# XChenZ/havatar

Hardware: AMD Instinct MI355X
Metric: rendered frames/sec @512^2, 64 samples/ray (higher is better)
Workload: dtype f32 emulated, full-width operands: every operand = hi + lo fp16 + tail (= the fp32 value itself, >= 24 significant bits); the three leading partial products on v_mfma_f32_32x32x16_f16, the three terms of order 2^-22 (hi.tail, tail.hi, lo.lo) on block-scaled 4-/6-bit v_mfma_scale_f32_32x32x64_f8f6f4

## Files before the change

### havatar_amd/_lib.py

```python
import ctypes as C
import os

from . import switches

_HERE = os.path.dirname(os.path.abspath(__file__))
LIB_PATH = os.path.join(_HERE, "lib", "libhavatar_hip.so")

HAV_F32, HAV_F16, HAV_BF16, HAV_F64 = 0, 1, 2, 3
HAV_MLP_SPLIT_BF16, HAV_MLP_F32, HAV_MLP_SPLIT_F16, HAV_MLP_SPLIT_F16_MX = 0, 1, 2, 3
ABI_VERSION = 8
HAV_FLAG_PAIR_KERNEL, HAV_FLAG_FINE_CACHE, HAV_FLAG_FINE_RECOMPUTE, HAV_FLAG_NO_FP16_GUARD = 1, 2, 4, 8
HAV_STATUS_FP16_FALLBACK = 1


class HavRenderParams(C.Structure):
    _fields_ = [("B", C.c_int32), ("R", C.c_int32), ("ray_stride", C.c_int32), ("S_c", C.c_int32),
                ("S_f", C.c_int32), ("perturb", C.c_int32), ("noise_std", C.c_float),
                ("plane_res", C.c_int32), ("plane_ch", C.c_int32), ("vol_res", C.c_int32),
                ("nerf_scale", C.c_float * 3), ("nerf_trans", C.c_float * 3),
                ("skin_scale", C.c_float * 3), ("skin_trans", C.c_float * 3),
                ("seed", C.c_uint64), ("rng_offset", C.c_uint64), ("mlp_mode", C.c_int32), ("flags", C.c_int32),
                ("rng_counter", C.c_void_p), ("workspace", C.c_void_p), ("workspace_bytes", C.c_uint64),
                ("dbg_zfine", C.c_void_p), ("status", C.c_void_p), ("grid_blocks", C.c_int32), ("reserved0", C.c_int32)]

# ... 160 lines not shown
    L.hav_upsample3d_2x_fwd.restype = i32
    L.hav_upsample3d_2x_bwd.argtypes = [vp, vp, i64, i32, i32, i32, vp]
    for fn in (L.hav_im2col3d, L.hav_col2im3d):
        fn.argtypes = [vp, vp, i32, i32, vp]
        fn.restype = i32
    L.hav_upsample3d_2x_bwd.restype = i32
    L.hav_mlp_train_blob_bytes.restype = i64
    L.hav_mlp_train_ops_bytes.argtypes = [i64]
    L.hav_mlp_train_ops_bytes.restype = i64
    L.hav_mlp_train_partial_bytes.argtypes = [i64]
    L.hav_mlp_train_partial_bytes.restype = i64
    L.hav_mlp_train_pack.argtypes = [vp, C.POINTER(HavMlpWeights), vp]
    L.hav_mlp_train_pack.restype = i32
    L.hav_mlp_train_fwd.argtypes = [vp, vp, vp, i64, vp]
    L.hav_mlp_train_fwd.restype = i32
    L.hav_mlp_train_bwd.argtypes = [vp, C.POINTER(HavMlpGrads), i32, vp, vp, vp, vp, vp, i64, vp]
    L.hav_mlp_train_bwd.restype = i32
    L.hav_mlp_train_fwd_xbf16.argtypes = [vp, vp, vp, i64, vp]
    L.hav_mlp_train_fwd_xbf16.restype = i32
    L.hav_mlp_train_bwd_xbf16.argtypes = [vp, C.POINTER(HavMlpGrads), i32, vp, vp, vp, vp, vp, i64, vp]
    L.hav_mlp_train_bwd_xbf16.restype = i32
    L.hav_triplane_prepare.argtypes = [vp, vp, vp, i32, i32, i32, i32, vp]
    L.hav_triplane_prepare.restype = i32
    L.hav_triplane_prepared_bytes.argtypes = [i32, i32, i32]
    L.hav_triplane_prepared_bytes.restype = i64
    L.hav_render_rays.argtypes = [C.POINTER(HavRenderParams)] + [vp] * 10 + [C.POINTER(HavRenderOut), vp]
    L.hav_render_rays.restype = i32
    L.hav_render_workspace_bytes.argtypes = [C.POINTER(HavRenderParams)]
    L.hav_render_workspace_bytes.restype = i64
    L.hav_render_variant_name.argtypes = [C.POINTER(HavRenderParams), i32, i32, C.c_char_p, i32]
    L.hav_render_variant_name.restype = i32
    L.hav_gen_rays.argtypes = [vp, i32, i32, C.POINTER(f32), C.POINTER(f32), f32, f32, i32, i32, vp]
    L.hav_gen_rays.restype = i32
    L.hav_debug_mlp_layer.argtypes = [vp, vp, vp, i32, i32, i64, vp]
    L.hav_debug_mlp_layer.restype = i32
    L.hav_conv3d_k3_packed_bytes.argtypes = [i32, i32]
    L.hav_conv3d_k3_packed_bytes.restype = i64
    for fn in (L.hav_conv3d_k3_pack, L.hav_conv3d_k3_pack_t):
        fn.argtypes = [vp, vp, i32, i32, f32, vp]
        fn.restype = i32
    L.hav_conv3d_k3_scratch_bytes.argtypes = [i32] * 6
    L.hav_conv3d_k3_scratch_bytes.restype = i64
    L.hav_conv3d_k3_fwd.argtypes = [vp] * 5 + [i32] * 6 + [vp, vp]
    L.hav_conv3d_k3_fwd.restype = i32
    L.hav_conv3d_k3_wgrad_scratch_bytes.argtypes = [i32] * 6
    L.hav_conv3d_k3_wgrad_scratch_bytes.restype = i64
# ... 30 lines not shown
```

### havatar_amd/csrc/hav_render.hip

```cpp
#include "hav_common.h"
#include <stdio.h>
#include <stdlib.h>
#include <string.h>
#include <atomic>

#define HAV_HID 128
#define HAV_PC 64
#define HAV_IN (2 * HAV_PC + 48)
#define KPE_STEPS 24
#define K2_STEPS (HAV_HID / 2)
#define OFF_W1PE 0
#define OFF_W2 (OFF_W1PE + KPE_STEPS * 4 * 64)
#define OFF_W4 (OFF_W2 + K2_STEPS * 4 * 64)
#define OFF_WFT (OFF_W4 + K2_STEPS * 2 * 4)
#define LDS_FLOATS (OFF_WFT + HAV_HID * 64)
#define OFF_B1 LDS_FLOATS
#define OFF_B2 (OFF_B1 + 128)
#define OFF_B4 (OFF_B2 + 128)
#define OFF_BF (OFF_B4 + 4)
#define OFF_W1F (OFF_BF + 64)
#define OFF_WFF (OFF_W1F + 2 * 128 * 64)
#define OFF_A1S (OFF_WFF + K2_STEPS * 2 * 64)
#define OFF_A2S (OFF_A1S + 3 * 4 * 3 * 64 * 4)
#define OFF_W4S (OFF_A2S + 8 * 4 * 3 * 64 * 4)
// ... 225 lines not shown
        al[d] |= ql << o;
        if (o + 6 > 32) al[d + 1] |= ql >> (32 - o);
    }
    unsigned int* rec = reinterpret_cast<unsigned int*>(blob) + OFF_MX + G * MX_G_DWORDS;
    for (int d = 0; d < 4; ++d) { rec[l * 4 + d] = ah[d]; rec[256 + l * 4 + d] = at[d]; rec[512 + l * 4 + d] = al[d]; }
    rec[768 + l * 2 + 0] = al[4]; rec[768 + l * 2 + 1] = al[5];
    rec[896 + l] = (unsigned int)(sh + 127) | ((unsigned int)(st + 127) << 8) | ((unsigned int)(sl_ + 127) << 16);
}

extern "C" int hav_mlp_pack(void* blob, const HavMlpWeights* w, void* stream)
{
    if (!blob || !w || !w->W1 || !w->b1 || !w->W2 || !w->b2 || !w->Wa || !w->ba || !w->Wf || !w->bf || !w->Wc || !w->bc)
        return HAV_EINVAL;
    hipLaunchKernelGGL(mlp_pack_kernel, dim3((BLOB_FLOATS + 255) / 256), dim3(256), 0, (hipStream_t)stream, (float*)blob, *w);
    HAV_LAUNCH_CHECK();
    hipLaunchKernelGGL(mlp_wmax_kernel, dim3(1), dim3(256), 0, (hipStream_t)stream, (float*)blob, *w);
    HAV_LAUNCH_CHECK();
    hipLaunchKernelGGL(mlp_pack_mx_kernel, dim3(MX_GROUPS), dim3(64), 0, (hipStream_t)stream, (float*)blob, *w);
    HAV_LAUNCH_CHECK();
    return 0;
}

#define PREP_TRAILER_WORDS 512
__global__ void __launch_bounds__(256) plane_project_kernel(float* __restrict__ dst, const float* __restrict__ src,
                                                            const float* __restrict__ blob, int HW, unsigned int* __restrict__ trailer)
{
    extern __shared__ __attribute__((aligned(16))) float sm[];
    float* sX = sm;
    float* sW = sm + 64 * 64;
    float* sO = sW + 128 * 65;
    const int pb = blockIdx.y;
    const int p = pb / (gridDim.y / 2);
    const int t0 = blockIdx.x * 64;
    const int tid = threadIdx.x, tx = tid & 63, ty = tid >> 6;
    const float* plane = src + (size_t)pb * HAV_PC * HW;
    for (int c = ty; c < HAV_PC; c += 4) sX[c * 64 + tx] = (t0 + tx < HW) ? plane[(size_t)c * HW + t0 + tx] : 0.f;
    const float* wsrc = blob + OFF_W1F + (size_t)p * 128 * 64;
    for (int i = tid; i < 128 * 64; i += 256) sW[(i >> 6) * 65 + (i & 63)] = wsrc[i];
    __syncthreads();
    float acc[32];
#pragma unroll
    for (int o = 0; o < 32; ++o) acc[o] = 0.f;
    for (int c = 0; c < HAV_PC; ++c) {
        const float xv = sX[c * 64 + tx];
#pragma unroll
        for (int o = 0; o < 32; ++o) acc[o] = fmaf(sW[(ty * 32 + o) * 65 + c], xv, acc[o]);
    }
#pragma unroll
    for (int o = 0; o < 32; ++o) sO[tx * 129 + ty * 32 + o] = acc[o];
    __syncthreads();
    float* out = dst + (size_t)pb * HW * 128;
    const int tg = p ? HAV_TG1 : HAV_TG;
    if (t0 + 64 <= HW && (64 >> tg) << tg == 64) {
        float4* blk = reinterpret_cast<float4*>(out + (size_t)(t0 >> tg) * (128 << tg));
        for (int q = tid; q < 64 * 32; q += 256) {
            const int g = q / (32 << tg), rem = q - g * (32 << tg);
            const int piece = rem >> tg, tx4 = rem & ((1 << tg) - 1);
            const float* so = sO + ((g << tg) + tx4) * 129 + 4 * piece;
            blk[q] = make_float4(so[0], so[1], so[2], so[3]);
        }
    } else {
        for (int i = tid; i < 64 * 128; i += 256) {
            const int t = i >> 7, hu = i & 127;
            const int tt = t0 + t;
            if (tt < HW) out[(size_t)(tt >> tg) * (128 << tg) + (hu >> 2) * (4 << tg) + (tt & ((1 << tg) - 1)) * 4 + (hu & 3)] = sO[t * 129 + hu];
        }
    }
    if (tid < 128) {
        float m = 0.f;
        unsigned int bad = 0;
        for (int t = 0; t < 64; ++t) {
            const float x = fabsf(sO[t * 129 + tid]);
            bad |= (x != x);
            m = fmaxf(m, x);
        }
        atomicMax(&trailer[p * 128 + tid], bad ? 0x7FC00000u : __float_as_uint(m));
    }
}

__global__ void __launch_bounds__(128) range_verdict_kernel(unsigned int* __restrict__ trailer, const float* __restrict__ blob)
{
    __shared__ float b1u[128], red[128];
    const int t = threadIdx.x;
    {
        const float bound = blob[OFF_RNG + t] + __uint_as_float(trailer[t]) + __uint_as_float(trailer[128 + t]);
        b1u[acc_row((t & 63) >> 4, t & 15, t >> 6)] = bound;
        red[t] = (bound < HAV_FP16_LIMIT) ? bound : __builtin_inff();
    }
    __syncthreads();
    for (int st = 64; st > 0; st >>= 1) { if (t < st) red[t] = fmaxf(red[t], red[t + st]); __syncthreads(); }
    const float m1 = red[0];
    __syncthreads();
    {
        const int m = t >> 5, l31 = t & 31;
        float bound = fabsf(blob[OFF_B2 + t]);
        for (int ks = 0; ks < K2_STEPS; ++ks)
            for (int hh = 0; hh < 2; ++hh)
                bound += fabsf(blob[OFF_W2 + (ks * 4 + m) * 64 + hh * 32 + l31]) * b1u[acc_row(ks >> 4, ks & 15, hh)];
        red[t] = (bound < HAV_FP16_LIMIT) ? bound : __builtin_inff();
    }
    __syncthreads();
    for (int st = 64; st > 0; st >>= 1) { if (t < st) red[t] = fmaxf(red[t], red[t + st]); __syncthreads(); }
    if (t == 0) {
        const float m2 = red[0], wmax = blob[OFF_RNG + 128];
        const bool safe = (m1 < HAV_FP16_LIMIT) && (m2 < HAV_FP16_LIMIT) && (wmax < HAV_FP16_LIMIT);
        trailer[256] = safe ? 0u : 1u;
        trailer[257] = __float_as_uint(m1);
        trailer[258] = __float_as_uint(m2);
    }
}

extern "C" int64_t hav_triplane_prepared_bytes(int B, int H, int W) { return ((int64_t)2 * B * H * W * 128 + PREP_TRAILER_WORDS) * 4; }

static bool attr_done(std::atomic<unsigned long long>& mask, int& dev)
{
    dev = 0;
    if (hipGetDevice(&dev) != hipSuccess || dev < 0 || dev > 63) dev = 0;
    return (mask.load(std::memory_order_acquire) >> dev) & 1ull;
}

extern "C" int hav_triplane_prepare(float* dst, const float* src_nchw, const void* mlp_blob, int B, int C, int H, int W,
                                    void* stream)
{
    if (!dst || !src_nchw || !mlp_blob || B < 1 || H < 1 || W < 1) return HAV_EINVAL;
    if (C != HAV_PC || (W & ((1 << HAV_TG) - 1)) || (W & ((1 << HAV_TG1) - 1))) return HAV_EUNSUP;
    const int HW = H * W;
    const size_t lds = (64 * 64 + 128 * 65 + 64 * 129) * sizeof(float);
    static std::atomic<unsigned long long> attr_mask{0};
    int dev;
    if (!attr_done(attr_mask, dev)) {
        hipError_t e = hipFuncSetAttribute((const void*)plane_project_kernel, hipFuncAttributeMaxDynamicSharedMemorySize, (int)lds);
        if (e != hipSuccess) return (int)e;
        attr_mask.fetch_or(1ull << dev, std::memory_order_release);
    }
    unsigned int* trailer = reinterpret_cast<unsigned int*>(dst + (size_t)2 * B * HW * 128);
    hipError_t me = hipMemsetAsync(trailer, 0, PREP_TRAILER_WORDS * 4, (hipStream_t)stream);
    if (me != hipSuccess) return (int)me;
    hipLaunchKernelGGL(plane_project_kernel, dim3((HW + 63) / 64, 2 * B), dim3(256), lds, (hipStream_t)stream, dst, src_nchw,
                       (const float*)mlp_blob, HW, trailer);
    HAV_LAUNCH_CHECK();
    hipLaunchKernelGGL(range_verdict_kernel, dim3(1), dim3(128), 0, (hipStream_t)stream, trailer, (const float*)mlp_blob);
    HAV_LAUNCH_CHECK();
    return 0;
}

#define DPP_QUAD_XOR1 0xB1
#define DPP_QUAD_XOR2 0x4E
#define DPP_ROW_SHR(n) (0x110 + (n))
#define DPP_ROW_MIRROR 0x140
#define DPP_ROW_HALF_MIRROR 0x141

template <int CTRL> __device__ __forceinline__ float dpp_mov(float old, float v)
{
    return __int_as_float(__builtin_amdgcn_update_dpp(__float_as_int(old), __float_as_int(v), CTRL, 0xf, 0xf, false));
}
__device__ __forceinline__ float row16_sum(float v)
{
    v += dpp_mov<DPP_QUAD_XOR1>(0.f, v);
    v += dpp_mov<DPP_QUAD_XOR2>(0.f, v);
    v += dpp_mov<DPP_ROW_HALF_MIRROR>(0.f, v);
    v += dpp_mov<DPP_ROW_MIRROR>(0.f, v);
    return v;
}
__device__ __forceinline__ float row16_max(float v)
// ... 1737 lines not shown
```

### havatar_amd/model/nerf_model.py

```python
import logging

import torch
import torch.nn as nn

from .network.embedder import get_embedder
from .styleUnet import StyleGAN_zxc
from .. import switches
from ..utils.sh_util import eval_sh
from ..utils.util import create_UniformBoxWarp, sample_from_triplane_new

_MLP_MODE_LOGGED = False


class _SplitKLinear(torch.autograd.Function):

    @staticmethod
    def forward(ctx, x, weight, bias):
        ctx.save_for_backward(x, weight)
        ctx.has_bias = bias is not None
        return torch.nn.functional.linear(x, weight, bias)

    @staticmethod
    def backward(ctx, dy):
        x, weight = ctx.saved_tensors
# ... 26 lines not shown
        self.pos_embedder, self.dim_xyz = get_embedder(multires=num_encoding_fn_xyz, input_dims=3, include_input=False)
        self.sh_deg = sh_deg
        self.use_sh = sh_deg >= 1
        include_xyz = self.dim_xyz if use_emb else 0
        self.dim_latent_code = 0 if cond_latent else latent_code_dim
        self.triPlane_feat_dim = triPlane_feat_dim
        self.rgb_feat_dim = rgb_feat_dim * (sh_deg + 1) ** 2
        self.use_emb, self.cond_latent, self.cond_c_dim = use_emb, cond_latent, cond_c_dim
        self.shared_backbone = self.two_head = False
        enc = dict(out_ch=triPlane_feat_dim, out_size=triplane_res, style_dim=latent_code_dim, middle_size=16, zero_latent=False,
                   zero_noise=True, no_skip=True, n_mlp=4, inp_size=256)
        self.XY_gen = StyleGAN_zxc(inp_ch=7, **enc)
        self.YZ_gen = StyleGAN_zxc(inp_ch=13, **enc)
        self.gridwarper = create_UniformBoxWarp(XYZ_bounding)
        self.layers_xyz = nn.ModuleList([nn.Linear(2 * triPlane_feat_dim + self.dim_latent_code + include_xyz, 128), nn.Linear(128, 128)])
        self.fc_alpha = nn.Linear(128, 1)
        self.fc_rgbFeat = nn.Linear(128, 64)
        self.fc_rgb = nn.Linear(64, self.rgb_feat_dim)
        self.relu = torch.nn.functional.relu
        self.triPlane_embeddings = None
        if not cond_latent:
            self.register_buffer("zero_latent", torch.zeros(latent_code_dim, dtype=torch.float32).reshape(1, -1))

    def set_conditional_embedding(self, **cond):
        styles = None
        if "latents" in cond:
            lat = cond["latents"]
            c = cond["cond_c"].reshape(lat.shape[0], -1)
            if self.cond_latent:
                styles = [torch.cat([lat, c], -1)] if self.cond_c_dim > 0 else [lat]
            else:
                styles = [self.zero_latent.expand(lat.shape[0], -1)]
        front, right = cond["front_render_cond"], cond["right_render_cond"]
        left = cond["left_render_cond"].flip(dims=[3])
        if left.shape[1] > 3:
            left = left[:, :-1]
        yz_in = torch.cat([left, right], dim=1)
        if front.is_cuda and not torch.is_grad_enabled() and switches.on("HAVATAR_ENC_STREAMS"):
            cur = torch.cuda.current_stream(front.device)
            side = self.__dict__.get("_side_stream")
            if side is None or side.device != front.device:
                side = self.__dict__["_side_stream"] = torch.cuda.Stream(device=front.device)
            side.wait_stream(cur)
            with torch.cuda.stream(side):
                yz, _ = self.YZ_gen(styles, yz_in)
            xy, _ = self.XY_gen(styles, front)
            cur.wait_stream(side)
            yz.record_stream(cur)
        else:
            xy, _ = self.XY_gen(styles, front)
            yz, _ = self.YZ_gen(styles, yz_in)
        self.triPlane_embeddings = torch.stack([xy, yz], dim=0)

    def sample_pts_triplane_feat(self, batch_pts, bidx=None):
        q = self.gridwarper(batch_pts)
        planes = self.triPlane_embeddings if bidx is None else self.triPlane_embeddings[:, bidx]
        if q.is_cuda and q.dtype == torch.float32 and q.ndim == 3 and planes.ndim == 5 and planes.shape[0] == 2 \
                and switches.on("HAVATAR_HIP_GATHER"):
            from ..native.gather import triplane_gather
            return triplane_gather(q, planes)
        f = sample_from_triplane_new(q, planes, padding_mode="zeros")
        return f.reshape(-1, f.shape[-1] * f.shape[-2])

    def forward(self, inp, pts_feat):
        xyz, dirs = inp[..., :3], inp[..., 3:]
        return self.mlp(torch.cat([pts_feat, self.pos_embedder(xyz)], -1), dirs)

    def mlp(self, x, dirs=None):
        if (x.is_cuda and x.dtype == torch.float32 and x.ndim == 2 and x.shape[1] == 176 and self.sh_deg == 0 and x.shape[0] >= 1024
                and torch.is_grad_enabled() and switches.choice("HAVATAR_TRAIN_MLP") == "bf16"):
            from ..native import mlp_train
            ws = self.mlp_tensors()
            if [tuple(w.shape) for w in ws] == mlp_train._SHAPES:
                global _MLP_MODE_LOGGED
                if not _MLP_MODE_LOGGED:
# ... 18 lines not shown
```

### havatar_amd/model/nerf_trainer.py

```python
import numpy as np
import torch
from einops import rearrange

from . import nerf_model
from .. import switches
from .Skinning_Field import Deformation_Field_new
from ..render import RayMarcher
from ..utils.nerf_util import sample_pdf, volume_render_radiance_field
from ..utils.training_util import get_minibatches
from ..utils.util import UniformBoxWarp_new, get_box_warp_param


_warned_wide_sampling = False


def _warn_wide_sampling(widest):
    global _warned_wide_sampling
    if _warned_wide_sampling:
        return
    _warned_wide_sampling = True
    import warnings
    warnings.warn("training with %d samples in a pass: the native compositing kernels hold 64, so this step takes the ATen statement of "
                  "the whole march.  Set HAVATAR_COMPOSITE_LONG=1 to keep it on the native route (up to 128 samples per pass)." % widest,
                  RuntimeWarning, stacklevel=3)


class Trainer(torch.nn.Module):
    def __init__(self, cfg, latent_codes_size=0, freeze_motion=True):
        super().__init__()
        self.cfg = cfg
        e = cfg.experiment
        self.latent_codes = torch.nn.Parameter(torch.zeros(latent_codes_size, e.latent_code_dim)) if latent_codes_size > 0 else None
        self.model_mode = e.model_mode
        latent_code_dim = e.latent_code_dim + (12 if e.cond_pose else 0) + (52 if e.cond_expr else 0)
        bounding = cfg.models.coarse.XYZ_bounding
        self.model_coarse = nerf_model.ConditionalTriplaneNeRFModel_multiRender_split_view(
            XYZ_bounding=bounding, triPlane_feat_dim=64, rgb_feat_dim=3, triplane_res=128, sh_deg=0,
            latent_code_dim=latent_code_dim, cond_c_dim=latent_code_dim - e.latent_code_dim)
        self.render_size, self.gen_size = cfg.models.StyleUnet.inp_size, cfg.models.StyleUnet.out_size
        b = {k: np.asarray(v, dtype=np.float64).copy() for k, v in zip("XYZ", bounding)}
        b["Y"][0] = 0.3 * b["Y"][1]
        scales, trans = get_box_warp_param(b["X"], b["Y"], b["Z"])
        self.headpose_skin_net = Deformation_Field_new(gridwarper=UniformBoxWarp_new(scales=scales, trans=trans))
        if freeze_motion:
            self.headpose_skin_net.requires_grad = False
        self._marcher = None

    def _hip_marcher(self):
        if self._marcher is None:
            gw, sw = self.model_coarse.gridwarper, self.headpose_skin_net.gridwarper
            f = lambda t: t.detach().reshape(3).cpu().tolist()
            self._marcher = RayMarcher(f(gw.scale_factor), f(gw.trans_factor), f(sw.scale_factor), f(sw.trans_factor))
        return self._marcher

    def nerf_forward(self, **inputs):
        cond_c = inputs["inv_head_T"].view(inputs["inv_head_T"].shape[0], -1)
        self.model_coarse.set_conditional_embedding(
            front_render_cond=inputs["front_render_cond"], left_render_cond=inputs["left_render_cond"],
            right_render_cond=inputs["right_render_cond"], latents=inputs["latent_code"], cond_c=cond_c)
        self._planes_dirty = True
        inv_head_T, ray_batch, background_prior = inputs["inv_head_T"], inputs["ray_batch"], inputs["background_prior"]
        mode = inputs["mode"]
        opt = getattr(self.cfg.nerf, mode)
        rd = ray_batch[..., 3:6]
        restore = [rd.shape[:-1] + (-1,), rd.shape[:-1], rd.shape[:-1], rd.shape[:-1]]
        if opt.num_fine > 0:
            restore += restore[:-1]
        if ray_batch.is_cuda:
            rays = ray_batch
        else:
            viewdirs = rd / rd.norm(p=2, dim=-1).unsqueeze(-1)
            rays = torch.cat((ray_batch, viewdirs), dim=-1)
        if self._use_hip(rays):
            self._decline_coarse = bool(inputs.get("_fine_maps_only", False)) and opt.num_fine > 0
            out = list(self.predict_and_render_radiance(mode, rays, background_prior, inv_head_T=inv_head_T))
            self._decline_coarse = False
        else:
            if rays.is_cuda:
                cap = max(switches.integer("HAVATAR_TRAIN_CHUNK_RAYS"), opt.chunksize)
                chunk = min(rays.shape[1], max(cap // rays.shape[0], 1))
            else:
                chunk = opt.chunksize // rays.shape[0]
            rb = get_minibatches(rays, chunksize=chunk, dim=1)
# ... 147 lines not shown
```

### havatar_amd/model/styleUnet.py

```python
import math
import random

import torch
from torch import nn
from torch.nn import functional as F

from .op import FusedLeakyReLU, conv2d_gradfix, fused_leaky_relu, upfirdn2d
from .. import switches
from ..graph import weights_epoch
from ..native import conv as _conv


def _fused_conv_enabled():
    return switches.on("HAVATAR_FUSED_CONV")


def _hip_train():
    return switches.on("HAVATAR_HIP_TRAIN")


def _conv_s2():
    return switches.on("HAVATAR_CONV_S2")


# ... 638 lines not shown
            out_channel = ch[2 ** i]
            self.convs.append(StyledConv(in_channel, out_channel, 3, self.style_dim, upsample=True, blur_kernel=blur_kernel))
            self.convs.append(StyledConv(out_channel, out_channel, 3, self.style_dim, blur_kernel=blur_kernel))
            self.to_rgbs.append(None if no_skip else ToRGB(out_channel, self.style_dim, out_channel=out_ch * 4, use_wt=False))
            in_channel = out_channel
        self.n_latent = self.log_size * 2 - (self.middle_log_size * 2 - 1) + 1 if n_latent is None else n_latent
        self.zero_noise = self.make_noise(zero_noise=True) if zero_noise else None
        if zero_latent:
            self.register_buffer("zero_latents", torch.zeros(1, self.n_latent, self.style_dim))
        else:
            self.zero_latents = None

    def make_noise(self, zero_noise=False):
        fn = torch.zeros if zero_noise else torch.randn
        noises = [torch.randn(1, 1, 2 ** self.middle_log_size, 2 ** self.middle_log_size)]
        for i in range(self.middle_log_size + 1, self.log_size + 1):
            noises += [fn(1, 1, 2 ** i, 2 ** i), fn(1, 1, 2 ** i, 2 ** i)]
        return noises

    def get_latent(self, styles, n_latent=None, inject_index=None):
        return _mix_latents([_run_style(self.style, s) for s in styles], self.n_latent if n_latent is None else n_latent, inject_index)

    def forward(self, styles, cond_feats, return_latents=False, inject_index=None, truncation=1, truncation_latent=None,
                input_is_latent=False, noise=None, randomize_noise=True, **kwargs):
        B = cond_feats.shape[0]
        if self.zero_latents is None:
            if not input_is_latent:
                assert self.n_mlp > 0
                styles = [_run_style(self.style, s) for s in styles]
            if truncation < 1:
                styles = [truncation_latent + truncation * (s - truncation_latent) for s in styles]
            latent = _mix_latents(styles, self.n_latent, inject_index)
        else:
            latent = self.zero_latents.expand(B, -1, -1)
        if self.zero_noise is not None:
            noise = [n.to(cond_feats.device) for n in self.zero_noise]
            self.zero_noise = noise
        elif noise is None:
            noise = [None] * self.num_layers if randomize_noise else [getattr(self.noises, f"noise_{i}") for i in range(self.num_layers)]

        pairs = [(self.conv1.conv, 0)] + ([] if self.no_skip else [(self.to_rgb1.conv, 1)])
        for k in range(len(self.convs) // 2):
            pairs += [(self.convs[2 * k].conv, 1 + 2 * k), (self.convs[2 * k + 1].conv, 2 + 2 * k)]
            if not self.no_skip:
                pairs.append((self.to_rgbs[k].conv, 3 + 2 * k))
        _prefetch_styles(self, pairs, latent)
        cond_list = self._encode(cond_feats)
        out = self.conv1(self.input(latent), latent[:, 0], noise=noise[0])
        skip = None if self.no_skip else self.to_rgb1(out, latent[:, 1])
        i = 1
        for conv_a, conv_b, n_a, n_b, to_rgb in zip(self.convs[::2], self.convs[1::2], noise[1::2], noise[2::2], self.to_rgbs):
            if 1 < i <= 2 * len(cond_list) + 1:
                out = self.comb_convs[-(i // 2)](torch.cat([out, cond_list[-(i // 2)]], dim=1))
            out = conv_b(conv_a(out, latent[:, i], noise=n_a), latent[:, i + 1], noise=n_b)
            if not self.no_skip:
                skip = to_rgb(out, latent[:, i + 2], skip)
            i += 2
        image = self.conv_out(out) if self.no_skip else skip
        return (image, latent) if return_latents else (image, None)


class SWGAN_unet(nn.Module, _CondEncoder):

    def __init__(self, inp_size, inp_ch, out_ch, out_size, style_dim, n_mlp, middle_size=8, c_dim=0, channel_multiplier=2,
                 blur_kernel=(1, 3, 3, 1), lr_mlp=0.01):
        super().__init__()
        self.inp_size, self.style_dim = inp_size, style_dim
        self.middle_log_size = int(math.log(middle_size, 2))
        self.style = _style_mlp(style_dim + c_dim, style_dim, n_mlp, lr_mlp)
        self.channels = ch = _CHANNELS(channel_multiplier)
        self.log_size = int(math.log(out_size, 2)) - 1

        in_channel = ch[inp_size // 2]
        self.from_rgbs, self.cond_convs, self.comb_convs = nn.ModuleList(), nn.ModuleList(), nn.ModuleList()
        self.comb_convs.append(ConvLayer(in_channel * 2, in_channel, 3))
        self.conv_in = ConvLayer(inp_ch, in_channel, 3, downsample=True)
        for i in range(int(math.log(inp_size, 2)) - 2, self.middle_log_size - 1, -1):
            out_channel = ch[2 ** i]
            self.from_rgbs.append(FromRGB(in_channel, inp_ch, downsample=True, use_wt=False))
            self.cond_convs.append(ConvBlock(in_channel, out_channel, blur_kernel))
            self.comb_convs.append(ConvLayer(out_channel * 2 if i > self.middle_log_size else out_channel, out_channel, 3))
            in_channel = out_channel
# ... 62 lines not shown
```

### havatar_amd/render.py

```python
import ctypes as C

import torch

from . import _lib, switches
from .graph import weights_epoch

_DEBUG_SYNC = switches.off("HAVATAR_DEBUG_SYNC")


def _ptr(t):
    return None if t is None else C.c_void_p(t.data_ptr())


def _stream():
    return C.c_void_p(torch.cuda.current_stream().cuda_stream)


def _chk_f32_cuda(name, t, allow_none=False):
    if t is None:
        if allow_none:
            return None
        raise RuntimeError(f"{name} is required")
    if not t.is_cuda:
        raise RuntimeError(f"{name} must be a CUDA/HIP tensor")
# ... 26 lines not shown
        self._workspace = None
        self.flags = 0
        if switches.choice("HAV_MARCH")[:1] == "p":
            self.flags |= _lib.HAV_FLAG_PAIR_KERNEL
        self.flags |= {"cache": _lib.HAV_FLAG_FINE_CACHE, "recompute": _lib.HAV_FLAG_FINE_RECOMPUTE}.get(switches.choice("HAV_FINE"), 0)
        self._status = None
        self.last_variant = None

    def set_mlp(self, W1, b1, W2, b2, Wa, ba, Wf, bf, Wc, bc, force=False):
        ts = [_chk_f32_cuda(n, t) for n, t in zip(("W1", "b1", "W2", "b2", "Wa", "ba", "Wf", "bf", "Wc", "bc"),
                                                   (W1, b1, W2, b2, Wa, ba, Wf, bf, Wc, bc))]
        key = tuple((t.data_ptr(), t._version) for t in ts) + (weights_epoch(),)
        if not force and key == self._blob_key and self.blob is not None:
            return
        L = _lib.lib()
        if self.blob is None or self.blob.device != ts[0].device:
            self.blob = torch.empty(int(L.hav_mlp_blob_bytes()) // 4, dtype=torch.float32, device=ts[0].device)
        w = _lib.HavMlpWeights(*[t.data_ptr() for t in ts])
        with torch.cuda.device(ts[0].device):
            _lib.check(L.hav_mlp_pack(_ptr(self.blob), C.byref(w), _stream()), "hav_mlp_pack")
        self._blob_key = key
        self._keep = ts

    def set_triplane(self, planes_nchw):
        if self.blob is None:
            raise RuntimeError("set_mlp() must be called before set_triplane()")
        p = _chk_f32_cuda("triPlane_embeddings", planes_nchw)
        two, B, Cc, H, W = p.shape
        if two != 2 or Cc != self.plane_ch or H != W:
            raise RuntimeError(f"unsupported tri-plane shape {tuple(p.shape)}")
        self.plane_res = H
        need = int(_lib.lib().hav_triplane_prepared_bytes(B, H, W)) // 4
        if self.planes_cl is None or self.planes_cl.numel() != need or self.planes_cl.device != p.device:
            self.planes_cl = torch.empty(need, dtype=torch.float32, device=p.device)
        self._planes_B = B
        with torch.cuda.device(p.device):
            _lib.check(_lib.lib().hav_triplane_prepare(_ptr(self.planes_cl), _ptr(p), _ptr(self.blob), B, Cc, H, W, _stream()),
                       "hav_triplane_prepare")
        self._planes_key = self._blob_key

    def render(self, rays, bg, inv_T, skin_vol, S_c, S_f, perturb=False, noise_std=0.0,
               t_rand=None, u_rand=None, noise_c=None, noise_f=None, dbg_zfine=False, coarse_outputs=True):
        if self.blob is None or self.planes_cl is None:
            raise RuntimeError("set_mlp() and set_triplane() must be called before render()")
        if self._planes_key != self._blob_key:
            raise RuntimeError("weights changed since set_triplane(): call set_triplane() again")
        rays = _chk_f32_cuda("ray_batch", rays)
        B, R, stride = rays.shape
        bg = _chk_f32_cuda("background_prior", bg, allow_none=True)
        inv_T = _chk_f32_cuda("inv_head_T", inv_T)
        vol = _chk_f32_cuda("canonical_W", skin_vol)
        if vol.dim() == 5:
            vol = vol[0]
        if self._planes_B != B or inv_T.shape[0] != B:
            raise RuntimeError("batch mismatch between rays, inv_head_T and the tri-plane")
        dev = rays.device
        S_fp = (S_c + 1) // 2 + S_f if S_f > 0 else 0
        p = _lib.HavRenderParams()
        p.B, p.R, p.ray_stride, p.S_c, p.S_f = B, R, stride, S_c, S_f
        p.perturb, p.noise_std = int(bool(perturb)), float(noise_std)
        p.plane_res, p.plane_ch, p.vol_res = self.plane_res, self.plane_ch, vol.shape[-1]
# ... 101 lines not shown
```

### include/havatar.h

```cpp
#ifndef HAVATAR_H
#define HAVATAR_H

#include <stdint.h>

#ifdef __cplusplus
extern "C" {
#endif

#define HAV_ABI_VERSION 8

#define HAV_EINVAL   (-1)
#define HAV_EUNSUP   (-2)

#define HAV_F32  0
#define HAV_F16  1
#define HAV_BF16 2
#define HAV_F64  3

int hav_abi_version(void);

int hav_fused_bias_act(void* out, const void* x, const void* b, const void* ref,
                       int dtype, int act, int grad, float alpha, float scale,
                       int64_t size_x, int64_t step_b, int64_t size_b, void* stream);

// ... 220 lines not shown
#define HAV_STATUS_FP16_FALLBACK 1u

#define HAV_MLP_SPLIT_BF16 0
#define HAV_MLP_F32        1
#define HAV_MLP_SPLIT_F16_MX 3
#define HAV_MLP_SPLIT_F16  2

int64_t hav_render_workspace_bytes(const HavRenderParams* p);

typedef struct HavMlpWeights {
    const float* W1; const float* b1;
    const float* W2; const float* b2;
    const float* Wa; const float* ba;
    const float* Wf; const float* bf;
    const float* Wc; const float* bc;
} HavMlpWeights;

int64_t hav_mlp_blob_bytes(void);
int hav_mlp_pack(void* blob, const HavMlpWeights* w, void* stream);

int64_t hav_triplane_prepared_bytes(int B, int H, int W);
int hav_triplane_prepare(float* dst, const float* src_nchw, const void* mlp_blob, int B, int C, int H, int W,
                         void* stream);

typedef struct HavRenderOut {
    float* rgb_coarse;
    float* depth_coarse;
    float* acc_coarse;
    float* weights_max;
    float* rgb_fine;
    float* depth_fine;
    float* acc_fine;
} HavRenderOut;

int hav_render_rays(const HavRenderParams* p, const float* rays, const float* bg,
                    const float* inv_T, const float* planes_prepared, const float* skin_vol,
                    const void* mlp_blob, const float* t_rand, const float* u_rand,
                    const float* noise_c, const float* noise_f, const HavRenderOut* out,
                    void* stream);

int hav_debug_mlp_layer(float* y, const float* x, const void* mlp_blob, int mlp_mode, int layer, int64_t n, void* stream);

int hav_render_variant_name(const HavRenderParams* p, int coarse_outputs, int injected_rand, char* buf, int len);

int hav_gen_rays(float* rays, int H, int W, const float intr[4], const float c2w[12],
                 float near, float far, int y0, int y1, void* stream);
// ... 6 lines not shown
```

Measured before the change: 116.0.

## Fuse plane bias+LeakyReLU with MFMA tri-plane projection in encoder handoff

Adds a handoff path in which each style-UNet output conv feeds a new MFMA-based plane projection kernel. That kernel applies the fused bias and LeakyReLU, writes the activated plane, and projects it through the first MLP layer in one pass. This removes the separate activation, the torch.stack copy and the re-read of planes in triplane_prepare. Per-block column maxima go to a scratch buffer and are reduced by a single verdict kernel instead of atomics. The default prepare path also switches from scalar FMAs to f32 MFMA. The cost is more API surface and a new scratch buffer, and the projection now accumulates in a different order on the fp32 MFMA.

```diff
diff --git a/havatar_amd/_lib.py b/havatar_amd/_lib.py
--- a/havatar_amd/_lib.py
+++ b/havatar_amd/_lib.py
@@ -206,6 +206,14 @@
     L.hav_mlp_train_bwd_xbf16.restype = i32
     L.hav_triplane_prepare.argtypes = [vp, vp, vp, i32, i32, i32, i32, vp]
     L.hav_triplane_prepare.restype = i32
+    L.hav_debug_plane_project_ref.argtypes = [vp, vp, vp, i32, i32, i32, i32, vp]
+    L.hav_debug_plane_project_ref.restype = i32
+    L.hav_plane_handoff_scratch_bytes.argtypes = [i32, i32, i32]
+    L.hav_plane_handoff_scratch_bytes.restype = i64
+    L.hav_plane_handoff.argtypes = [vp, vp, vp, vp, C.c_float, C.c_float, vp, vp, i32, i32, i32, i32, i32, vp]
+    L.hav_plane_handoff.restype = i32
+    L.hav_plane_verdict.argtypes = [vp, vp, vp, i32, i32, i32, vp]
+    L.hav_plane_verdict.restype = i32
     L.hav_triplane_prepared_bytes.argtypes = [i32, i32, i32]
     L.hav_triplane_prepared_bytes.restype = i64
     L.hav_render_rays.argtypes = [C.POINTER(HavRenderParams)] + [vp] * 10 + [C.POINTER(HavRenderOut), vp]
diff --git a/havatar_amd/csrc/hav_render.hip b/havatar_amd/csrc/hav_render.hip
--- a/havatar_amd/csrc/hav_render.hip
+++ b/havatar_amd/csrc/hav_render.hip
@@ -271,6 +271,40 @@
 }
 
 #define PREP_TRAILER_WORDS 512
+__device__ __forceinline__ void plane_project_store(float* __restrict__ dst, const float* sO, int pb, int p, int t0, int tid, int HW,
+                                                    unsigned int* __restrict__ trailer, unsigned int* __restrict__ rows)
+{
+    float* out = dst + (size_t)pb * HW * 128;
+    const int tg = p ? HAV_TG1 : HAV_TG;
+    if (t0 + 64 <= HW && (64 >> tg) << tg == 64) {
+        float4* blk = reinterpret_cast<float4*>(out + (size_t)(t0 >> tg) * (128 << tg));
+        for (int q = tid; q < 64 * 32; q += 256) {
+            const int g = q / (32 << tg), rem = q - g * (32 << tg);
+            const int piece = rem >> tg, tx4 = rem & ((1 << tg) - 1);
+            const float* so = sO + ((g << tg) + tx4) * 129 + 4 * piece;
+            blk[q] = make_float4(so[0], so[1], so[2], so[3]);
+        }
+    } else {
+        for (int i = tid; i < 64 * 128; i += 256) {
+            const int t = i >> 7, hu = i & 127;
+            const int tt = t0 + t;
+            if (tt < HW) out[(size_t)(tt >> tg) * (128 << tg) + (hu >> 2) * (4 << tg) + (tt & ((1 << tg) - 1)) * 4 + (hu & 3)] = sO[t * 129 + hu];
+        }
+    }
+    if (tid < 128) {
+        float m = 0.f;
+        unsigned int bad = 0;
+        for (int t = 0; t < 64; ++t) {
+            const float x = fabsf(sO[t * 129 + tid]);
+            bad |= (x != x);
+            m = fmaxf(m, x);
+        }
+        const unsigned int word = bad ? 0x7FC00000u : __float_as_uint(m);
+        if (rows) rows[((size_t)pb * gridDim.x + blockIdx.x) * 128 + tid] = word;
+        else atomicMax(&trailer[p * 128 + tid], word);
+    }
+}
+
 __global__ void __launch_bounds__(256) plane_project_kernel(float* __restrict__ dst, const float* __restrict__ src,
                                                             const float* __restrict__ blob, int HW, unsigned int* __restrict__ trailer)
 {
@@ -298,41 +332,71 @@
 #pragma unroll
     for (int o = 0; o < 32; ++o) sO[tx * 129 + ty * 32 + o] = acc[o];
     __syncthreads();
-    float* out = dst + (size_t)pb * HW * 128;
-    const int tg = p ? HAV_TG1 : HAV_TG;
-    if (t0 + 64 <= HW && (64 >> tg) << tg == 64) {
-        float4* blk = reinterpret_cast<float4*>(out + (size_t)(t0 >> tg) * (128 << tg));
-        for (int q = tid; q < 64 * 32; q += 256) {
-            const int g = q / (32 << tg), rem = q - g * (32 << tg);
-            const int piece = rem >> tg, tx4 = rem & ((1 << tg) - 1);
-            const float* so = sO + ((g << tg) + tx4) * 129 + 4 * piece;
-            blk[q] = make_float4(so[0], so[1], so[2], so[3]);
+    plane_project_store(dst, sO, pb, p, t0, tid, HW, trailer, nullptr);
+}
+
+struct PlaneAct { const float* bias; float* act; float slope, gain; int p0; };
+template <bool HANDOFF>
+__global__ void __launch_bounds__(256) plane_project_mfma_kernel(float* __restrict__ dst, const float* __restrict__ src,
+                                                                 const float* __restrict__ blob, int HW, int B, unsigned int* __restrict__ trailer,
+                                                                 unsigned int* __restrict__ rows, PlaneAct pa)
+{
+    __shared__ __attribute__((aligned(16))) float sm[64 * 129];
+    float* sX = sm;
+    float* sO = sm;
+    const int pb = HANDOFF ? pa.p0 * B + blockIdx.y : blockIdx.y;
+    const int p = pb / B;
+    const int t0 = blockIdx.x * 64;
+    const int tid = threadIdx.x, lane = tid & 63, wv = tid >> 6, j = lane & 31, h = lane >> 5;
+    const float* plane = src + (size_t)(HANDOFF ? blockIdx.y : pb) * HAV_PC * HW;
+    if (HANDOFF) {
+        float* act = pa.act + (size_t)pb * HAV_PC * HW;
+        for (int c = wv; c < HAV_PC; c += 4) {
+            float y = 0.f;
+            if (t0 + lane < HW) {
+                const float x = plane[(size_t)c * HW + t0 + lane] + pa.bias[c];
+                y = ((x > 0.f) ? x : x * pa.slope) * pa.gain;
+                act[(size_t)c * HW + t0 + lane] = y;
+            }
+            sX[c * 64 + lane] = y;
         }
     } else {
-        for (int i = tid; i < 64 * 128; i += 256) {
-            const int t = i >> 7, hu = i & 127;
-            const int tt = t0 + t;
-            if (tt < HW) out[(size_t)(tt >> tg) * (128 << tg) + (hu >> 2) * (4 << tg) + (tt & ((1 << tg) - 1)) * 4 + (hu & 3)] = sO[t * 129 + hu];
-        }
-    }
-    if (tid < 128) {
-        float m = 0.f;
-        unsigned int bad = 0;
-        for (int t = 0; t < 64; ++t) {
-            const float x = fabsf(sO[t * 129 + tid]);
-            bad |= (x != x);
-            m = fmaxf(m, x);
-        }
-        atomicMax(&trailer[p * 128 + tid], bad ? 0x7FC00000u : __float_as_uint(m));
-    }
-}
-
-__global__ void __launch_bounds__(128) range_verdict_kernel(unsigned int* __restrict__ trailer, const float* __restrict__ blob)
-{
-    __shared__ float b1u[128], red[128];
-    const int t = threadIdx.x;
-    {
-        const float bound = blob[OFF_RNG + t] + __uint_as_float(trailer[t]) + __uint_as_float(trailer[128 + t]);
+        for (int c = wv; c < HAV_PC; c += 4) sX[c * 64 + lane] = (t0 + lane < HW) ? plane[(size_t)c * HW + t0 + lane] : 0.f;
+    }
+    const float4* wrow = reinterpret_cast<const float4*>(blob + OFF_W1F + (size_t)p * 128 * 64 + (size_t)(32 * wv + j) * 64);
+    float a[32];
+#pragma unroll
+    for (int i = 0; i < 16; ++i) {
+        const float4 q = wrow[i];
+        a[2 * i] = h ? q.y : q.x;
+        a[2 * i + 1] = h ? q.w : q.z;
+    }
+    __syncthreads();
+    f32x16 acc0, acc1;
+#pragma unroll
+    for (int r = 0; r < 16; ++r) { acc0[r] = 0.f; acc1[r] = 0.f; }
+#pragma unroll
+    for (int ks = 0; ks < 32; ++ks) {
+        const float b0 = sX[(2 * ks + h) * 64 + j], b1 = sX[(2 * ks + h) * 64 + 32 + j];
+        acc0 = __builtin_amdgcn_mfma_f32_32x32x2f32(a[ks], b0, acc0, 0, 0, 0);
+        acc1 = __builtin_amdgcn_mfma_f32_32x32x2f32(a[ks], b1, acc1, 0, 0, 0);
+    }
+    __syncthreads();
+#pragma unroll
+    for (int r = 0; r < 16; ++r) {
+        const int hu = 32 * wv + (r & 3) + 8 * (r >> 2) + 4 * h;
+        sO[j * 129 + hu] = acc0[r];
+        sO[(32 + j) * 129 + hu] = acc1[r];
+    }
+    __syncthreads();
+    plane_project_store(dst, sO, pb, p, t0, tid, HW, trailer, rows);
+}
+
+__device__ __forceinline__ void range_verdict_body(unsigned int* __restrict__ trailer, const float* __restrict__ blob, float c0, float c1, int t,
+                                                   float* b1u, float* red)
+{
+    if (t < 128) {
+        const float bound = blob[OFF_RNG + t] + c0 + c1;
         b1u[acc_row((t & 63) >> 4, t & 15, t >> 6)] = bound;
         red[t] = (bound < HAV_FP16_LIMIT) ? bound : __builtin_inff();
     }
@@ -340,7 +404,7 @@
     for (int st = 64; st > 0; st >>= 1) { if (t < st) red[t] = fmaxf(red[t], red[t + st]); __syncthreads(); }
     const float m1 = red[0];
     __syncthreads();
-    {
+    if (t < 128) {
         const int m = t >> 5, l31 = t & 31;
         float bound = fabsf(blob[OFF_B2 + t]);
         for (int ks = 0; ks < K2_STEPS; ++ks)
@@ -359,6 +423,42 @@
     }
 }
 
+__global__ void __launch_bounds__(128) range_verdict_kernel(unsigned int* __restrict__ trailer, const float* __restrict__ blob)
+{
+    __shared__ float b1u[128], red[128];
+    const int t = threadIdx.x;
+    range_verdict_body(trailer, blob, __uint_as_float(trailer[t]), __uint_as_float(trailer[128 + t]), t, b1u, red);
+}
+
+__global__ void __launch_bounds__(1024) range_verdict_rows_kernel(unsigned int* __restrict__ trailer, const float* __restrict__ blob,
+                                                                  const unsigned int* __restrict__ rows, int nrows)
+{
+    __shared__ unsigned int part[8][256];
+    __shared__ float b1u[128], red[128];
+    const int t = threadIdx.x, hu = t & 127, sl = t >> 7;
+    for (int p = 0; p < 2; ++p) {
+        const unsigned int* col = rows + (size_t)p * nrows * 128 + hu;
+        unsigned int m = 0, m1 = 0, m2 = 0, m3 = 0;
+        int r = sl;
+        for (; r + 24 < nrows; r += 32) {
+            const unsigned int a0 = col[(size_t)r * 128], a1 = col[(size_t)(r + 8) * 128], a2 = col[(size_t)(r + 16) * 128],
+                               a3 = col[(size_t)(r + 24) * 128];
+            m = max(m, a0); m1 = max(m1, a1); m2 = max(m2, a2); m3 = max(m3, a3);
+        }
+        for (; r < nrows; r += 8) m = max(m, col[(size_t)r * 128]);
+        part[sl][p * 128 + hu] = max(max(m, m1), max(m2, m3));
+    }
+    __syncthreads();
+    if (t < 256) {
+        unsigned int m = part[0][t];
+        for (int q = 1; q < 8; ++q) m = max(m, part[q][t]);
+        part[0][t] = m;
+        trailer[t] = m;
+    }
+    __syncthreads();
+    range_verdict_body(trailer, blob, __uint_as_float(part[0][hu]), __uint_as_float(part[0][128 + hu]), t, b1u, red);
+}
+
 extern "C" int64_t hav_triplane_prepared_bytes(int B, int H, int W) { return ((int64_t)2 * B * H * W * 128 + PREP_TRAILER_WORDS) * 4; }
 
 static bool attr_done(std::atomic<unsigned long long>& mask, int& dev)
@@ -368,27 +468,71 @@
     return (mask.load(std::memory_order_acquire) >> dev) & 1ull;
 }
 
-extern "C" int hav_triplane_prepare(float* dst, const float* src_nchw, const void* mlp_blob, int B, int C, int H, int W,
-                                    void* stream)
+static int triplane_prepare_impl(float* dst, const float* src_nchw, const void* mlp_blob, int B, int C, int H, int W, void* stream, bool ref)
 {
     if (!dst || !src_nchw || !mlp_blob || B < 1 || H < 1 || W < 1) return HAV_EINVAL;
     if (C != HAV_PC || (W & ((1 << HAV_TG) - 1)) || (W & ((1 << HAV_TG1) - 1))) return HAV_EUNSUP;
     const int HW = H * W;
-    const size_t lds = (64 * 64 + 128 * 65 + 64 * 129) * sizeof(float);
-    static std::atomic<unsigned long long> attr_mask{0};
-    int dev;
-    if (!attr_done(attr_mask, dev)) {
-        hipError_t e = hipFuncSetAttribute((const void*)plane_project_kernel, hipFuncAttributeMaxDynamicSharedMemorySize, (int)lds);
-        if (e != hipSuccess) return (int)e;
-        attr_mask.fetch_or(1ull << dev, std::memory_order_release);
-    }
     unsigned int* trailer = reinterpret_cast<unsigned int*>(dst + (size_t)2 * B * HW * 128);
-    hipError_t me = hipMemsetAsync(trailer, 0, PREP_TRAILER_WORDS * 4, (hipStream_t)stream);
-    if (me != hipSuccess) return (int)me;
-    hipLaunchKernelGGL(plane_project_kernel, dim3((HW + 63) / 64, 2 * B), dim3(256), lds, (hipStream_t)stream, dst, src_nchw,
-                       (const float*)mlp_blob, HW, trailer);
+    if (ref) {
+        const size_t lds = (64 * 64 + 128 * 65 + 64 * 129) * sizeof(float);
+        static std::atomic<unsigned long long> attr_mask{0};
+        int dev;
+        if (!attr_done(attr_mask, dev)) {
+            hipError_t e = hipFuncSetAttribute((const void*)plane_project_kernel, hipFuncAttributeMaxDynamicSharedMemorySize, (int)lds);
+            if (e != hipSuccess) return (int)e;
+            attr_mask.fetch_or(1ull << dev, std::memory_order_release);
+        }
+        hipError_t me = hipMemsetAsync(trailer, 0, PREP_TRAILER_WORDS * 4, (hipStream_t)stream);
+        if (me != hipSuccess) return (int)me;
+        hipLaunchKernelGGL(plane_project_kernel, dim3((HW + 63) / 64, 2 * B), dim3(256), lds, (hipStream_t)stream, dst, src_nchw,
+                           (const float*)mlp_blob, HW, trailer);
+    } else {
+        hipError_t me = hipMemsetAsync(trailer, 0, PREP_TRAILER_WORDS * 4, (hipStream_t)stream);
+        if (me != hipSuccess) return (int)me;
+        hipLaunchKernelGGL(plane_project_mfma_kernel<false>, dim3((HW + 63) / 64, 2 * B), dim3(256), 0, (hipStream_t)stream, dst, src_nchw,
+                           (const float*)mlp_blob, HW, B, trailer, (unsigned int*)nullptr, PlaneAct{nullptr, nullptr, 0.f, 0.f, 0});
+    }
     HAV_LAUNCH_CHECK();
     hipLaunchKernelGGL(range_verdict_kernel, dim3(1), dim3(128), 0, (hipStream_t)stream, trailer, (const float*)mlp_blob);
+    HAV_LAUNCH_CHECK();
+    return 0;
+}
+
+extern "C" int hav_triplane_prepare(float* dst, const float* src_nchw, const void* mlp_blob, int B, int C, int H, int W,
+                                    void* stream)
+{
+    return triplane_prepare_impl(dst, src_nchw, mlp_blob, B, C, H, W, stream, false);
+}
+
+extern "C" int hav_debug_plane_project_ref(float* dst, const float* src_nchw, const void* mlp_blob, int B, int C, int H, int W,
+                                           void* stream)
+{
+    return triplane_prepare_impl(dst, src_nchw, mlp_blob, B, C, H, W, stream, true);
+}
+
+extern "C" int64_t hav_plane_handoff_scratch_bytes(int B, int H, int W) { return (int64_t)2 * B * ((H * W + 63) / 64) * 128 * 4; }
+
+extern "C" int hav_plane_handoff(float* dst, float* planes_nchw, const float* raw, const float* bias, float slope, float gain,
+                                 const void* mlp_blob, void* scratch, int p, int B, int C, int H, int W, void* stream)
+{
+    if (!dst || !planes_nchw || !raw || !bias || !mlp_blob || !scratch || p < 0 || p > 1 || B < 1 || H < 1 || W < 1) return HAV_EINVAL;
+    if (C != HAV_PC || (W & ((1 << HAV_TG) - 1)) || (W & ((1 << HAV_TG1) - 1))) return HAV_EUNSUP;
+    const int HW = H * W;
+    unsigned int* trailer = reinterpret_cast<unsigned int*>(dst + (size_t)2 * B * HW * 128);
+    hipLaunchKernelGGL(plane_project_mfma_kernel<true>, dim3((HW + 63) / 64, B), dim3(256), 0, (hipStream_t)stream, dst, raw,
+                       (const float*)mlp_blob, HW, B, trailer, (unsigned int*)scratch, PlaneAct{bias, planes_nchw, slope, gain, p});
+    HAV_LAUNCH_CHECK();
+    return 0;
+}
+
+extern "C" int hav_plane_verdict(float* dst, const void* scratch, const void* mlp_blob, int B, int H, int W, void* stream)
+{
+    if (!dst || !scratch || !mlp_blob || B < 1 || H < 1 || W < 1) return HAV_EINVAL;
+    const int HW = H * W;
+    unsigned int* trailer = reinterpret_cast<unsigned int*>(dst + (size_t)2 * B * HW * 128);
+    hipLaunchKernelGGL(range_verdict_rows_kernel, dim3(1), dim3(1024), 0, (hipStream_t)stream, trailer, (const float*)mlp_blob,
+                       (const unsigned int*)scratch, B * ((HW + 63) / 64));
     HAV_LAUNCH_CHECK();
     return 0;
 }
diff --git a/havatar_amd/model/nerf_model.py b/havatar_amd/model/nerf_model.py
--- a/havatar_amd/model/nerf_model.py
+++ b/havatar_amd/model/nerf_model.py
@@ -72,7 +72,7 @@
         if not cond_latent:
             self.register_buffer("zero_latent", torch.zeros(latent_code_dim, dtype=torch.float32).reshape(1, -1))
 
-    def set_conditional_embedding(self, **cond):
+    def set_conditional_embedding(self, handoff=None, **cond):
         styles = None
         if "latents" in cond:
             lat = cond["latents"]
@@ -82,10 +82,21 @@
             else:
                 styles = [self.zero_latent.expand(lat.shape[0], -1)]
         front, right = cond["front_render_cond"], cond["right_render_cond"]
-        left = cond["left_render_cond"].flip(dims=[3])
-        if left.shape[1] > 3:
-            left = left[:, :-1]
-        yz_in = torch.cat([left, right], dim=1)
+
+        def yz_input():
+            left = cond["left_render_cond"].flip(dims=[3])
+            if left.shape[1] > 3:
+                left = left[:, :-1]
+            return torch.cat([left, right], dim=1)
+        planes = None
+        if (handoff is not None and front.is_cuda and front.dtype == torch.float32 and not torch.is_grad_enabled()
+                and self.XY_gen.handoff_ok(front) and self.YZ_gen.handoff_ok(front)
+                and self.XY_gen.conv_out[0].weight.shape[0] == self.YZ_gen.conv_out[0].weight.shape[0] == handoff.plane_ch):
+            res = 2 ** self.XY_gen.log_size
+            if 2 ** self.YZ_gen.log_size == res and res % 4 == 0:
+                planes = handoff.handoff_begin(front.shape[0], res, res, front.device)
+        hx = None if planes is None else (handoff, planes, 0)
+        hy = None if planes is None else (handoff, planes, 1)
         if front.is_cuda and not torch.is_grad_enabled() and switches.on("HAVATAR_ENC_STREAMS"):
             cur = torch.cuda.current_stream(front.device)
             side = self.__dict__.get("_side_stream")
@@ -93,14 +104,20 @@
                 side = self.__dict__["_side_stream"] = torch.cuda.Stream(device=front.device)
             side.wait_stream(cur)
             with torch.cuda.stream(side):
-                yz, _ = self.YZ_gen(styles, yz_in)
-            xy, _ = self.XY_gen(styles, front)
+                yz, _ = self.YZ_gen(styles, yz_input(), handoff=hy)
+            xy, _ = self.XY_gen(styles, front, handoff=hx)
             cur.wait_stream(side)
-            yz.record_stream(cur)
+            if planes is None:
+                yz.record_stream(cur)
         else:
-            xy, _ = self.XY_gen(styles, front)
-            yz, _ = self.YZ_gen(styles, yz_in)
+            xy, _ = self.XY_gen(styles, front, handoff=hx)
+            yz, _ = self.YZ_gen(styles, yz_input(), handoff=hy)
+        if planes is not None:
+            handoff.handoff_end(planes)
+            self.triPlane_embeddings = planes
+            return True
         self.triPlane_embeddings = torch.stack([xy, yz], dim=0)
+        return False
 
     def sample_pts_triplane_feat(self, batch_pts, bidx=None):
         q = self.gridwarper(batch_pts)
diff --git a/havatar_amd/model/nerf_trainer.py b/havatar_amd/model/nerf_trainer.py
--- a/havatar_amd/model/nerf_trainer.py
+++ b/havatar_amd/model/nerf_trainer.py
@@ -45,6 +45,7 @@
         if freeze_motion:
             self.headpose_skin_net.requires_grad = False
         self._marcher = None
+        self.plane_handoff = True
 
     def _hip_marcher(self):
         if self._marcher is None:
@@ -55,10 +56,17 @@
 
     def nerf_forward(self, **inputs):
         cond_c = inputs["inv_head_T"].view(inputs["inv_head_T"].shape[0], -1)
-        self.model_coarse.set_conditional_embedding(
-            front_render_cond=inputs["front_render_cond"], left_render_cond=inputs["left_render_cond"],
+        marcher = None
+        if (getattr(self, "plane_handoff", True) and inputs["ray_batch"].is_cuda and not torch.is_grad_enabled() and self.model_coarse.sh_deg == 0):
+            marcher = self._hip_marcher()
+            marcher.set_mlp(*[t.detach() for t in self.model_coarse.mlp_tensors()])
+        handed = self.model_coarse.set_conditional_embedding(
+            handoff=marcher, front_render_cond=inputs["front_render_cond"], left_render_cond=inputs["left_render_cond"],
             right_render_cond=inputs["right_render_cond"], latents=inputs["latent_code"], cond_c=cond_c)
         self._planes_dirty = True
+        if handed:
+            planes = self.model_coarse.triPlane_embeddings
+            self._planes_key, self._planes_dirty = (planes.data_ptr(), planes._version, marcher._blob_key), False
         inv_head_T, ray_batch, background_prior = inputs["inv_head_T"], inputs["ray_batch"], inputs["background_prior"]
         mode = inputs["mode"]
         opt = getattr(self.cfg.nerf, mode)
diff --git a/havatar_amd/model/styleUnet.py b/havatar_amd/model/styleUnet.py
--- a/havatar_amd/model/styleUnet.py
+++ b/havatar_amd/model/styleUnet.py
@@ -684,7 +684,7 @@
         return _mix_latents([_run_style(self.style, s) for s in styles], self.n_latent if n_latent is None else n_latent, inject_index)
 
     def forward(self, styles, cond_feats, return_latents=False, inject_index=None, truncation=1, truncation_latent=None,
-                input_is_latent=False, noise=None, randomize_noise=True, **kwargs):
+                input_is_latent=False, noise=None, randomize_noise=True, handoff=None, **kwargs):
         B = cond_feats.shape[0]
         if self.zero_latents is None:
             if not input_is_latent:
@@ -718,8 +718,20 @@
             if not self.no_skip:
                 skip = to_rgb(out, latent[:, i + 2], skip)
             i += 2
-        image = self.conv_out(out) if self.no_skip else skip
+        if handoff is not None and self.handoff_ok(out):
+            marcher, planes, p = handoff
+            act = self.conv_out[1]
+            marcher.handoff_plane(p, self.conv_out[0](out), act.bias, act.negative_slope, act.scale, planes)
+            image = planes[p]
+        else:
+            image = self.conv_out(out) if self.no_skip else skip
         return (image, latent) if return_latents else (image, None)
+
+    def handoff_ok(self, x):
+        co = getattr(self, "conv_out", None)
+        return (self.no_skip and co is not None and len(co) == 2 and isinstance(co[0], EqualConv2d) and isinstance(co[1], FusedLeakyReLU)
+                and co[1].bias is not None and co[0].weight.shape[-1] == 1 and x.is_cuda and x.dtype == torch.float32
+                and not torch.is_grad_enabled() and not switches.off("HAVATAR_CONV_1X1"))
 
 
 class SWGAN_unet(nn.Module, _CondEncoder):
diff --git a/havatar_amd/render.py b/havatar_amd/render.py
--- a/havatar_amd/render.py
+++ b/havatar_amd/render.py
@@ -72,7 +72,7 @@
         self._blob_key = key
         self._keep = ts
 
-    def set_triplane(self, planes_nchw):
+    def set_triplane(self, planes_nchw, ref=False):
         if self.blob is None:
             raise RuntimeError("set_mlp() must be called before set_triplane()")
         p = _chk_f32_cuda("triPlane_embeddings", planes_nchw)
@@ -85,8 +85,41 @@
             self.planes_cl = torch.empty(need, dtype=torch.float32, device=p.device)
         self._planes_B = B
         with torch.cuda.device(p.device):
-            _lib.check(_lib.lib().hav_triplane_prepare(_ptr(self.planes_cl), _ptr(p), _ptr(self.blob), B, Cc, H, W, _stream()),
-                       "hav_triplane_prepare")
+            fn = _lib.lib().hav_debug_plane_project_ref if ref else _lib.lib().hav_triplane_prepare
+            _lib.check(fn(_ptr(self.planes_cl), _ptr(p), _ptr(self.blob), B, Cc, H, W, _stream()), "hav_triplane_prepare")
+        self._planes_key = self._blob_key
+
+    def handoff_begin(self, B, H, W, device):
+        if self.blob is None:
+            raise RuntimeError("set_mlp() must be called before handoff_begin()")
+        L = _lib.lib()
+        self.plane_res = H
+        need = int(L.hav_triplane_prepared_bytes(B, H, W)) // 4
+        if self.planes_cl is None or self.planes_cl.numel() != need or self.planes_cl.device != device:
+            self.planes_cl = torch.empty(need, dtype=torch.float32, device=device)
+        rows = int(L.hav_plane_handoff_scratch_bytes(B, H, W)) // 4
+        hr = getattr(self, "_handoff_rows", None)
+        if hr is None or hr.numel() != rows or hr.device != device:
+            self._handoff_rows = torch.empty(rows, dtype=torch.int32, device=device)
+        self._planes_key = None
+        return torch.empty(2, B, self.plane_ch, H, W, dtype=torch.float32, device=device)
+
+    def handoff_plane(self, p, raw, bias, slope, gain, planes):
+        raw, bias = _chk_f32_cuda("raw", raw), _chk_f32_cuda("bias", bias)
+        B, Cc, H, W = raw.shape
+        if tuple(planes.shape) != (2, B, Cc, H, W) or Cc != self.plane_ch or bias.numel() != Cc:
+            raise RuntimeError(f"handoff_plane: raw {tuple(raw.shape)} does not fit planes {tuple(planes.shape)}")
+        with torch.cuda.device(raw.device):
+            _lib.check(_lib.lib().hav_plane_handoff(_ptr(self.planes_cl), _ptr(planes), _ptr(raw), _ptr(bias), float(slope), float(gain),
+                                                    _ptr(self.blob), _ptr(self._handoff_rows), int(p), B, Cc, H, W, _stream()),
+                       "hav_plane_handoff")
+
+    def handoff_end(self, planes):
+        _, B, _, H, W = planes.shape
+        with torch.cuda.device(planes.device):
+            _lib.check(_lib.lib().hav_plane_verdict(_ptr(self.planes_cl), _ptr(self._handoff_rows), _ptr(self.blob), B, H, W, _stream()),
+                       "hav_plane_verdict")
+        self._planes_B = B
         self._planes_key = self._blob_key
 
     def render(self, rays, bg, inv_T, skin_vol, S_c, S_f, perturb=False, noise_std=0.0,
diff --git a/include/havatar.h b/include/havatar.h
--- a/include/havatar.h
+++ b/include/havatar.h
@@ -266,6 +266,13 @@
 int64_t hav_triplane_prepared_bytes(int B, int H, int W);
 int hav_triplane_prepare(float* dst, const float* src_nchw, const void* mlp_blob, int B, int C, int H, int W,
                          void* stream);
+int hav_debug_plane_project_ref(float* dst, const float* src_nchw, const void* mlp_blob, int B, int C, int H, int W,
+                                void* stream);
+
+int64_t hav_plane_handoff_scratch_bytes(int B, int H, int W);
+int hav_plane_handoff(float* dst, float* planes_nchw, const float* raw, const float* bias, float slope, float gain,
+                      const void* mlp_blob, void* scratch, int p, int B, int C, int H, int W, void* stream);
+int hav_plane_verdict(float* dst, const void* scratch, const void* mlp_blob, int B, int H, int W, void* stream);
 
 typedef struct HavRenderOut {
     float* rgb_coarse;
```

Result: no change. 115.0 (-0.9%).
